# DeNA/Chainer_Realtime_Multi-Person_Pose_Estimation

Hardware: AMD Instinct MI355X
Metric: frames/sec at 368x368 batch (1/2/4/8 GPU) + keypoint-match vs reference (higher is better)
Workload: dtype f32; 1 GPU; batch32_368x368_synthetic_uint8_per_gpu; per_gpu_batch=32, global_batch=32, map=320x320, weights=seeded He + calibrated head, records_gathered=32, status_bits=0

## Files before the change

### chainer_realtime_multi-person_pose_estimation_amd/csrc/conv1_wino.hip

```cpp
#include <type_traits>
#include "pmx_common.h"
#include "wino_util.h"

#ifndef PMX_C1W_ABLATE
#define PMX_C1W_ABLATE 0
#endif
namespace {
constexpr int TT = 8;
constexpr int HW1 = 2 * TT + 2;
constexpr int NPX = HW1 * HW1;
constexpr int PW = HW1 + 2, PPX = PW * PW;
constexpr int LDA = 68;
constexpr int LDU = 36;
constexpr int U_HALF = 4 * 64 * LDU;
constexpr int RAW_ELEMS = NPX * LDA, U_ELEMS = 2 * U_HALF;
constexpr int LDS_BYTES = (RAW_ELEMS + U_ELEMS + 64) * 4;
static_assert(LDS_BYTES <= 160 * 1024, "conv1 Winograd kernel: LDS");
static_assert(PPX * 3 <= U_ELEMS, "the input patch lives in U before the first transform");
}

__global__ __launch_bounds__(256, 1) void conv1_wino_kernel(const ConvArgs a)
{
    extern __shared__ float4 smem4[];
    float* const s_raw = reinterpret_cast<float*>(smem4);
    float* const s_u = s_raw + RAW_ELEMS;
    float* const s_bias = s_u + U_ELEMS;
    float* const s_patch = s_u;
    const int tid = threadIdx.x, lane = tid & 63, wave = tid >> 6, li = lane & 31, kh = lane >> 5;
    const int th = wave >> 1, chh = wave & 1;
    int tile;
    {
        const int nwg = gridDim.x, bid = blockIdx.x;
        const int q = nwg >> 3, r = nwg & 7, xcd = bid & 7, loc = bid >> 3;
        tile = (xcd < r ? xcd * (q + 1) : r * (q + 1) + (xcd - r) * q) + loc;
    }
    int H = a.H, W = a.W, s_tiles_x = a.tiles_x, tiles_per_img = a.tiles_x * a.tiles_y;
    size_t s_pix_in = 0, s_pix_out = 0;
    if (a.nseg > 0) {
        int sg = 0;
        for (int k = 1; k < a.nseg; ++k) sg = tile >= a.segs[k].tile0 ? k : sg;
        const ConvSeg S = a.segs[sg];
        H = S.H; W = S.W; s_tiles_x = S.tiles_x; tiles_per_img = S.tiles_img;
        s_pix_in = (size_t)(unsigned)S.pix0; s_pix_out = (size_t)(unsigned)S.pixo;
        tile -= S.tile0;
    }
    const int bimg = tile / tiles_per_img;
    const int trem = tile - bimg * tiles_per_img;
    const int y0 = (trem / s_tiles_x) * (2 * TT), x0 = (trem % s_tiles_x) * (2 * TT);
    constexpr int OUTSIDE = (int)0x80000000;

    if (a.g[1].in) {
        const uint8_t* src8 = reinterpret_cast<const uint8_t*>(a.g[1].in) + (s_pix_in + (size_t)bimg * H * W) * 3;
        const __amdgpu_buffer_rsrc_t irsrc = __builtin_amdgcn_make_buffer_rsrc(const_cast<uint8_t*>(src8), 0, (unsigned)(H * W * 3), 0x00020000);
        const float divisor = __builtin_bit_cast(float, (unsigned)a.kbounds);
        unsigned char pb[2][3];
        bool pin[2];
#pragma unroll
        for (int r = 0; r < 2; ++r) {
            const int f = tid + r * 256;
            const int py = f / PW, px = f - py * PW;
            const int gy = y0 - 2 + py, gx = x0 - 2 + px;
            pin[r] = f < PPX && (unsigned)gy < (unsigned)H && (unsigned)gx < (unsigned)W;
            const int o = pin[r] ? (gy * W + gx) * 3 : OUTSIDE;
#pragma unroll
            for (int ch = 0; ch < 3; ++ch) pb[r][ch] = __builtin_amdgcn_raw_buffer_load_b8(irsrc, o, ch, 0);
        }
#pragma unroll
        for (int r = 0; r < 2; ++r) {
            const int f = tid + r * 256;
            if (f < PPX) {
#pragma unroll
                for (int ch = 0; ch < 3; ++ch)
                    s_patch[f * 3 + ch] = pin[r] ? __fsub_rn(__fdiv_rn((float)pb[r][ch], divisor), 0.5f) : 0.f;
            }
        }
    } else {
        const __amdgpu_buffer_rsrc_t irsrc = __builtin_amdgcn_make_buffer_rsrc(const_cast<float*>(a.g[0].in + (s_pix_in + (size_t)bimg * H * W) * a.lda), 0,
                                                                               (unsigned)(H * W * a.lda) * 4u, 0x00020000);
        float4 pv[2];
#pragma unroll
        for (int r = 0; r < 2; ++r) {
            const int f = tid + r * 256;
            const int py = f / PW, px = f - py * PW;
            const int gy = y0 - 2 + py, gx = x0 - 2 + px;
            const bool in = f < PPX && (unsigned)gy < (unsigned)H && (unsigned)gx < (unsigned)W;
            pv[r] = __builtin_bit_cast(float4, __builtin_amdgcn_raw_buffer_load_b128(irsrc, in ? (gy * W + gx) * a.lda * 4 : OUTSIDE, 0, 0));
        }
#pragma unroll
        for (int r = 0; r < 2; ++r) {
            const int f = tid + r * 256;
            if (f < PPX) { s_patch[f * 3 + 0] = pv[r].x; s_patch[f * 3 + 1] = pv[r].y; s_patch[f * 3 + 2] = pv[r].z; }
        }
    }
    float wv[14];
    int koff[14];
    {
        const float* wp = a.g[1].w + chh * (14 * 64) + lane;
#pragma unroll
        for (int s = 0; s < 14; ++s) {
            const int k = 2 * s + kh, kk = k < 27 ? k : 26;
            wv[s] = (PMX_C1W_ABLATE & 32) ? 1.f : wp[s * 64];
            const int tap = kk / 3;
            koff[s] = ((tap / 3) * PW + tap % 3) * 3 + kk % 3;
        }
    }
    f32x4 b1[4];
#pragma unroll
    for (int q = 0; q < 4; ++q) b1[q] = *reinterpret_cast<const f32x4*>(a.g[1].bias + chh * 32 + 8 * q + 4 * kh);
    if (tid < 64) s_bias[tid] = a.g[0].bias[tid];
    const __amdgpu_buffer_rsrc_t wrsrc = __builtin_amdgcn_make_buffer_rsrc(const_cast<float*>(a.g[0].w), 0, 0x7fffffff, 0x00020000);
    const unsigned b_off = (unsigned)((chh * 1024 + li * 8 + kh * 4) * 4);
    constexpr unsigned panel_b = 64u * 32u * 4u, freq_b = panel_b * 2u;
    auto wload = [&](int g) -> f32x4 {
        const int P = g >> 4, s = g & 15;
        const unsigned so = (unsigned)(4 * (P & 3) + (s >> 2)) * freq_b + (unsigned)(P >> 2) * panel_b;
        return __builtin_bit_cast(f32x4, __builtin_amdgcn_raw_buffer_load_b128(wrsrc, b_off + (unsigned)(s & 3) * 1024u, so, 0));
    };
    f32x4 bw[16];
#pragma unroll
    for (int g = 0; g < 8; ++g) bw[g] = wload(g);
    __syncthreads();

    const float b1s = a.g[1].bias[chh * 32 + li];
    int c1_m[5], c1_pb[5];
    float c1_hi[5];
#pragma unroll
    for (int i = 0; i < 5; ++i) {
        const int m = ((wave >> 1) + 2 * i) * 32 + li;
        const int hy = m / HW1, hx = m - hy * HW1;
        c1_m[i] = m;
        c1_pb[i] = (hy * PW + hx) * 3;
        const int gy = y0 - 1 + hy, gx = x0 - 1 + hx;
        c1_hi[i] = ((unsigned)gy < (unsigned)H && (unsigned)gx < (unsigned)W) ? __builtin_inff() : 0.f;
    }
    if (!(PMX_C1W_ABLATE & 1)) {
        const f32x16 z16 = {0.f, 0.f, 0.f, 0.f, 0.f, 0.f, 0.f, 0.f, 0.f, 0.f, 0.f, 0.f, 0.f, 0.f, 0.f, 0.f};
        float pa[2][14];
        f32x16 acc1[2];
        f32x4 ev;
#pragma unroll
        for (int sg = 0; sg < 14; ++sg) pa[0][sg] = s_patch[c1_pb[0] + koff[sg]];
        auto c1_finish = [&](const f32x16& acc, int i, int sg) {
            const int q = sg / 3, part = sg - 3 * q;
            if (q >= 4) return;
            if (part == 0) ev = pk_add4(f32x4{acc[4 * q], acc[4 * q + 1], acc[4 * q + 2], acc[4 * q + 3]}, b1[q]);
            else if (part == 1) {
#pragma unroll
                for (int e = 0; e < 4; ++e) ev[e] = __builtin_amdgcn_fmed3f(ev[e], 0.f, c1_hi[i]);
            } else *reinterpret_cast<f32x4*>(&s_raw[c1_m[i] * LDA + chh * 32 + 8 * q + 4 * kh]) = ev;
        };
#pragma unroll
        for (int i = 0; i < 5; ++i) {
#pragma unroll
            for (int sg = 0; sg < 14; ++sg) {
                acc1[i & 1] = __builtin_amdgcn_mfma_f32_32x32x2f32(wv[sg], pa[i & 1][sg], sg == 0 ? z16 : acc1[i & 1], 0, 0, 0);
                if (i + 1 < 5) pa[(i + 1) & 1][sg] = s_patch[c1_pb[i + 1] + koff[sg]];
                if (i > 0) c1_finish(acc1[(i - 1) & 1], i - 1, sg);
                __builtin_amdgcn_sched_barrier(0);
            }
        }
        {
            const int p4 = 2 * (wave >> 1) + kh, m = 320 + p4;
            const int hy = m / HW1, hx = m - hy * HW1, pb = (hy * PW + hx) * 3;
            float accv = 0.f;
#pragma unroll
            for (int sg = 0; sg < 14; ++sg) {
                const float other = __shfl_xor(wv[sg], 32);
                const float we = kh ? other : wv[sg], wo = kh ? wv[sg] : other;
                const int k0 = 2 * sg, k1 = 2 * sg + 1;
                accv = __builtin_fmaf(s_patch[pb + ((k0 / 9) * PW + (k0 / 3) % 3) * 3 + k0 % 3], we, accv);
                if (k1 < 27) accv = __builtin_fmaf(s_patch[pb + ((k1 / 9) * PW + (k1 / 3) % 3) * 3 + k1 % 3], wo, accv);
            }
            const int gy = y0 - 1 + hy, gx = x0 - 1 + hx;
            const float hi = ((unsigned)gy < (unsigned)H && (unsigned)gx < (unsigned)W) ? __builtin_inff() : 0.f;
            s_raw[m * LDA + chh * 32 + li] = __builtin_amdgcn_fmed3f(accv + b1s, 0.f, hi);
        }
#pragma unroll
        for (int sg = 0; sg < 12; ++sg) c1_finish(acc1[0], 4, sg);
    }
    __syncthreads();

    const int tg = tid >> 3, tc = tid & 7;
    const int tt = (tg & ~7) + ((tg & 7) >> 1) + 4 * (tg & 1);
    int t_raw[2];
#pragma unroll
    for (int it = 0; it < 2; ++it) {
        const int t = tt + 32 * it;
        t_raw[it] = ((2 * (t >> 3)) * HW1 + 2 * (t & 7)) * LDA + tc * 4;
    }
    const int t_u = tt * LDU + tc * 4;
    auto row_a = [](int i) { return i == 0 ? 0 : i == 1 ? 1 : i == 2 ? 2 : 1; };
    auto row_b = [](int i) { return i == 0 ? 2 : i == 1 ? 2 : i == 2 ? 1 : 3; };
    f32x4 dA[2][4], dB[2][4], wq[2][4], vq[2][4];
    auto tr_read = [&](int it, int k, int ch, int i) {
        const int row = k < 4 ? row_a(i) : row_b(i), jx = k & 3;
        const f32x4 v = *reinterpret_cast<const f32x4*>(&s_raw[t_raw[it] + (row * HW1 + jx) * LDA + ch * 32]);
        if (k < 4) dA[it][jx] = v; else dB[it][jx] = v;
    };
    auto tr_w = [&](int it, int jx, int i) { wq[it][jx] = i == 1 ? pk_add4(dA[it][jx], dB[it][jx]) : pk_sub4(dA[it][jx], dB[it][jx]); };
    auto tr_v = [&](int it, int jv) {
        vq[it][jv] = jv == 0 ? pk_sub4(wq[it][0], wq[it][2]) : jv == 1 ? pk_add4(wq[it][1], wq[it][2]) : jv == 2 ? pk_sub4(wq[it][2], wq[it][1]) : pk_sub4(wq[it][1], wq[it][3]);
    };
    auto tr_store = [&](int it, int jv, int half) {
        *reinterpret_cast<f32x4*>(&s_u[half * U_HALF + (jv * 64 + 32 * it) * LDU + t_u]) = vq[it][jv];
    };
    auto side = [&](int t, int ch, int i, int half) {
        if (t < 8) tr_read(0, t, ch, i);
        else if (t < 16) {
            tr_read(1, t - 8, ch, i);
            if (t < 12) tr_w(0, t - 8, i); else tr_v(0, t - 12);
        } else if (t < 20) { tr_store(0, t - 16, half); tr_w(1, t - 16, i); }
        else if (t < 24) tr_v(1, t - 20);
        else if (t < 28) tr_store(1, t - 24, half);
    };
#pragma unroll
    for (int t = 0; t < 28; ++t) side(t, 0, 0, 0);
    __syncthreads();

    f32x16 acc[16];
    f32x4 av[4];
    const int a_off = (32 * th + li) * LDU + kh * 4;
    av[0] = *reinterpret_cast<const f32x4*>(&s_u[a_off]);
    av[1] = *reinterpret_cast<const f32x4*>(&s_u[a_off + 8]);
    const f32x16 zero16 = {0.f, 0.f, 0.f, 0.f, 0.f, 0.f, 0.f, 0.f, 0.f, 0.f, 0.f, 0.f, 0.f, 0.f, 0.f, 0.f};
    auto phase = [&](auto P_c) {
        constexpr int P = decltype(P_c)::value;
        constexpr int ch = P >> 2, i = P & 3, half = P & 1;
        constexpr int Pn = P + 1, chn = Pn >> 2, in = Pn & 3, halfn = Pn & 1;
#pragma unroll
        for (int s = 0; s < 16; ++s) {
            const int f = 4 * i + (s >> 2), g = P * 16 + s;
#pragma unroll
            for (int e = 0; e < 4; ++e) {
                acc[f] = wino_mfma(av[s & 3][e], bw[g & 15][e], (ch == 0 && (s & 3) == 0 && e == 0) ? zero16 : acc[f]);
                if (e == 0) {
                    if (g + 8 < 128 && !(PMX_C1W_ABLATE & 4)) bw[(g + 8) & 15] = wload(g + 8);
                    if (s == 14 && P < 7) __syncthreads();
                    __builtin_amdgcn_sched_barrier(0);
                } else if (e == 1) {
                    const int sn = s + 2;
                    if (sn < 16) av[sn & 3] = *reinterpret_cast<const f32x4*>(&s_u[half * U_HALF + ((sn >> 2) * 64) * LDU + a_off + (sn & 3) * 8]);
                    else if (P < 7) av[sn & 3] = *reinterpret_cast<const f32x4*>(&s_u[halfn * U_HALF + a_off + (sn & 3) * 8]);
                    __builtin_amdgcn_sched_barrier(0);
                } else {
                    if (P < 7 && !(PMX_C1W_ABLATE & 2)) side(2 * s + (e - 2), chn, in, halfn);
                    __builtin_amdgcn_sched_barrier(0);
                }
            }
        }
    };
    if (!(PMX_C1W_ABLATE & 8)) {
    phase(std::integral_constant<int, 0>{}); phase(std::integral_constant<int, 1>{}); phase(std::integral_constant<int, 2>{});
    phase(std::integral_constant<int, 3>{}); phase(std::integral_constant<int, 4>{}); phase(std::integral_constant<int, 5>{});
    phase(std::integral_constant<int, 6>{}); phase(std::integral_constant<int, 7>{});
    } else {
#pragma unroll
        for (int f = 0; f < 16; ++f) acc[f] = zero16;
    }
    __builtin_amdgcn_sched_barrier(0);
#pragma unroll
    for (int f = 0; f < 16; ++f) asm volatile("" : "+a"(acc[f]));
    __builtin_amdgcn_sched_barrier(0);

    f32x4 bq[4];
#pragma unroll
    for (int q = 0; q < 4; ++q) bq[q] = *reinterpret_cast<const f32x4*>(&s_bias[chh * 32 + 8 * q + 4 * kh]);
    float pooled[16];
#pragma unroll
    for (int rp = 0; rp < 8; ++rp) {
        f32x2 t0[4], t1[4];
#pragma unroll
        for (int j = 0; j < 4; ++j) {
            const f32x2 m0 = {acc[0 + j][2 * rp], acc[0 + j][2 * rp + 1]}, m1 = {acc[4 + j][2 * rp], acc[4 + j][2 * rp + 1]};
            const f32x2 m2 = {acc[8 + j][2 * rp], acc[8 + j][2 * rp + 1]}, m3 = {acc[12 + j][2 * rp], acc[12 + j][2 * rp + 1]};
            t0[j] = pk_add2(pk_add2(m0, m1), m2);
            t1[j] = pk_sub2(pk_sub2(m1, m2), m3);
        }
        const f32x2 o0 = pk_add2(pk_add2(t0[0], t0[1]), t0[2]), o1 = pk_sub2(pk_sub2(t0[1], t0[2]), t0[3]);
        const f32x2 o2 = pk_add2(pk_add2(t1[0], t1[1]), t1[2]), o3 = pk_sub2(pk_sub2(t1[1], t1[2]), t1[3]);
#pragma unroll
        for (int h2 = 0; h2 < 2; ++h2) pooled[2 * rp + h2] = fmaxf(fmaxf(o0[h2], o1[h2]), fmaxf(o2[h2], o3[h2]));
    }
    const int Hp = H >> 1, Wp = W >> 1, ldc_b = a.ldc * 4;
    const __amdgpu_buffer_rsrc_t orsrc = __builtin_amdgcn_make_buffer_rsrc(a.g[0].out + (s_pix_out + (size_t)bimg * Hp * Wp) * a.ldc, 0, (unsigned)(Hp * Wp * ldc_b), 0x00020000);
    const int tb = 32 * th + li;
    const int py = (y0 >> 1) + (tb >> 3), px = (x0 >> 1) + (tb & 7);
    const int o = (py < Hp && px < Wp) ? (int)__umul24(__umul24(py, Wp) + px, ldc_b) + (chh * 32 + 4 * kh) * 4 : OUTSIDE;
    const float lo = a.relu ? 0.f : -__builtin_inff();
    typedef unsigned u32x4 __attribute__((ext_vector_type(4)));
#pragma unroll
    for (int q = 0; q < 4; ++q) {
        f32x4 v;
#pragma unroll
        for (int e = 0; e < 4; ++e) v[e] = fmaxf(pooled[4 * q + e] + bq[q][e], lo);
        if (PMX_C1W_ABLATE & 16) asm volatile("" :: "v"(v));
        else __builtin_amdgcn_raw_buffer_store_b128(__builtin_bit_cast(u32x4, v), orsrc, o + q * 32, 0, 0);
    }
}

int conv1_wino_launch(const ConvArgs& a0, hipStream_t stream)
{
    ConvArgs a = a0;
    PMX_CHECK(a.cout_pad == 64 && a.g[0].cout == 64 && a.nch == 4 && a.lda >= 4 && a.pool && a.ldc % 4 == 0, PMX_ERR_INVALID,
              "conv1 winograd: needs conv1_2 = 64 -> 64 with the pool and a >= 4-channel padded input");
    PMX_CHECK(a.H % 2 == 0 && a.W % 2 == 0, PMX_ERR_INVALID, "conv: pooled layer needs even H, W");
    PMX_CHECK((long long)a.H * a.W * a.lda * 4 < (1ll << 31) && (long long)a.H * a.W * a.ldc < (1ll << 31), PMX_ERR_INVALID, "conv: image too large for 32-bit offsets");
    a.tiles_x = (a.W + 2 * TT - 1) / (2 * TT);
    a.tiles_y = (a.H + 2 * TT - 1) / (2 * TT);
    a.ksplit = 1;
    if (!a.g[1].in) a.kbounds = 0;
    static bool attr_set[PMX_MAX_DEVICES] = {};
    if (int rc = conv_allow_big_lds(reinterpret_cast<const void*>(conv1_wino_kernel), attr_set)) return rc;
    PMX_CHECK(a.nseg == 0 || (a.segs && a.seg_tiles > 0), PMX_ERR_INVALID, "conv1 winograd: segments without a table");
    hipLaunchKernelGGL(conv1_wino_kernel, dim3(a.nseg ? (unsigned)a.seg_tiles : (unsigned)(a.tiles_x * a.tiles_y * a.B)), dim3(256), LDS_BYTES, stream, a);
    PMX_HIP(hipGetLastError());
    return PMX_OK;
}
```

Baseline: 960.1 frames/s.

## Swizzle conv1 raw tile LDS layout, issue weight loads before patch staging

Drops the padded LDA=68 row stride for an unpadded stride of 64 with an XOR swizzle of the 16-byte chunk index. The conv1 MFMA stores and the Winograd transform reads both use it, keeping LDS access conflict-free while shrinking the buffer. The filter-transform weight prefetch now issues before the input patch load so their latencies overlap. The scalar tail for pixels 320-323 is replaced by an extra MFMA tile on waves with th==0. This adds redundant MFMA work on half the waves, creates wave divergence, and makes the index math more complex.

New measurement: 955.6 frames/s. No clear change (-0.5%).

```diff
diff --git a/chainer_realtime_multi-person_pose_estimation_amd/csrc/conv1_wino.hip b/chainer_realtime_multi-person_pose_estimation_amd/csrc/conv1_wino.hip
--- a/chainer_realtime_multi-person_pose_estimation_amd/csrc/conv1_wino.hip
+++ b/chainer_realtime_multi-person_pose_estimation_amd/csrc/conv1_wino.hip
@@ -10,13 +10,15 @@
 constexpr int HW1 = 2 * TT + 2;
 constexpr int NPX = HW1 * HW1;
 constexpr int PW = HW1 + 2, PPX = PW * PW;
-constexpr int LDA = 68;
+constexpr int LDA = 64;
+constexpr int NT1 = (NPX + 31) / 32;
 constexpr int LDU = 36;
 constexpr int U_HALF = 4 * 64 * LDU;
 constexpr int RAW_ELEMS = NPX * LDA, U_ELEMS = 2 * U_HALF;
 constexpr int LDS_BYTES = (RAW_ELEMS + U_ELEMS + 64) * 4;
 static_assert(LDS_BYTES <= 160 * 1024, "conv1 Winograd kernel: LDS");
 static_assert(PPX * 3 <= U_ELEMS, "the input patch lives in U before the first transform");
+__device__ __forceinline__ int c1w_swz(int m) { return ((m & 1) << 2) | (m & 2) | (((m >> 2) & 1) * 9); }
 }
 
 __global__ __launch_bounds__(256, 1) void conv1_wino_kernel(const ConvArgs a)
@@ -26,7 +28,7 @@
     float* const s_u = s_raw + RAW_ELEMS;
     float* const s_bias = s_u + U_ELEMS;
     float* const s_patch = s_u;
-    const int tid = threadIdx.x, lane = tid & 63, wave = tid >> 6, li = lane & 31, kh = lane >> 5;
+    const int tid = threadIdx.x, lane = tid & 63, wave = __builtin_amdgcn_readfirstlane(tid >> 6), li = lane & 31, kh = lane >> 5;
     const int th = wave >> 1, chh = wave & 1;
     int tile;
     {
@@ -49,49 +51,6 @@
     const int y0 = (trem / s_tiles_x) * (2 * TT), x0 = (trem % s_tiles_x) * (2 * TT);
     constexpr int OUTSIDE = (int)0x80000000;
 
-    if (a.g[1].in) {
-        const uint8_t* src8 = reinterpret_cast<const uint8_t*>(a.g[1].in) + (s_pix_in + (size_t)bimg * H * W) * 3;
-        const __amdgpu_buffer_rsrc_t irsrc = __builtin_amdgcn_make_buffer_rsrc(const_cast<uint8_t*>(src8), 0, (unsigned)(H * W * 3), 0x00020000);
-        const float divisor = __builtin_bit_cast(float, (unsigned)a.kbounds);
-        unsigned char pb[2][3];
-        bool pin[2];
-#pragma unroll
-        for (int r = 0; r < 2; ++r) {
-            const int f = tid + r * 256;
-            const int py = f / PW, px = f - py * PW;
-            const int gy = y0 - 2 + py, gx = x0 - 2 + px;
-            pin[r] = f < PPX && (unsigned)gy < (unsigned)H && (unsigned)gx < (unsigned)W;
-            const int o = pin[r] ? (gy * W + gx) * 3 : OUTSIDE;
-#pragma unroll
-            for (int ch = 0; ch < 3; ++ch) pb[r][ch] = __builtin_amdgcn_raw_buffer_load_b8(irsrc, o, ch, 0);
-        }
-#pragma unroll
-        for (int r = 0; r < 2; ++r) {
-            const int f = tid + r * 256;
-            if (f < PPX) {
-#pragma unroll
-                for (int ch = 0; ch < 3; ++ch)
-                    s_patch[f * 3 + ch] = pin[r] ? __fsub_rn(__fdiv_rn((float)pb[r][ch], divisor), 0.5f) : 0.f;
-            }
-        }
-    } else {
-        const __amdgpu_buffer_rsrc_t irsrc = __builtin_amdgcn_make_buffer_rsrc(const_cast<float*>(a.g[0].in + (s_pix_in + (size_t)bimg * H * W) * a.lda), 0,
-                                                                               (unsigned)(H * W * a.lda) * 4u, 0x00020000);
-        float4 pv[2];
-#pragma unroll
-        for (int r = 0; r < 2; ++r) {
-            const int f = tid + r * 256;
-            const int py = f / PW, px = f - py * PW;
-            const int gy = y0 - 2 + py, gx = x0 - 2 + px;
-            const bool in = f < PPX && (unsigned)gy < (unsigned)H && (unsigned)gx < (unsigned)W;
-            pv[r] = __builtin_bit_cast(float4, __builtin_amdgcn_raw_buffer_load_b128(irsrc, in ? (gy * W + gx) * a.lda * 4 : OUTSIDE, 0, 0));
-        }
-#pragma unroll
-        for (int r = 0; r < 2; ++r) {
-            const int f = tid + r * 256;
-            if (f < PPX) { s_patch[f * 3 + 0] = pv[r].x; s_patch[f * 3 + 1] = pv[r].y; s_patch[f * 3 + 2] = pv[r].z; }
-        }
-    }
     float wv[14];
     int koff[14];
     {
@@ -107,7 +66,7 @@
     f32x4 b1[4];
 #pragma unroll
     for (int q = 0; q < 4; ++q) b1[q] = *reinterpret_cast<const f32x4*>(a.g[1].bias + chh * 32 + 8 * q + 4 * kh);
-    if (tid < 64) s_bias[tid] = a.g[0].bias[tid];
+    const float b2v = a.g[0].bias[tid & 63];
     const __amdgpu_buffer_rsrc_t wrsrc = __builtin_amdgcn_make_buffer_rsrc(const_cast<float*>(a.g[0].w), 0, 0x7fffffff, 0x00020000);
     const unsigned b_off = (unsigned)((chh * 1024 + li * 8 + kh * 4) * 4);
     constexpr unsigned panel_b = 64u * 32u * 4u, freq_b = panel_b * 2u;
@@ -119,16 +78,61 @@
     f32x4 bw[16];
 #pragma unroll
     for (int g = 0; g < 8; ++g) bw[g] = wload(g);
+    __builtin_amdgcn_sched_barrier(0);
+    if (a.g[1].in) {
+        const uint8_t* src8 = reinterpret_cast<const uint8_t*>(a.g[1].in) + (s_pix_in + (size_t)bimg * H * W) * 3;
+        const __amdgpu_buffer_rsrc_t irsrc = __builtin_amdgcn_make_buffer_rsrc(const_cast<uint8_t*>(src8), 0, (unsigned)(H * W * 3), 0x00020000);
+        const float divisor = __builtin_bit_cast(float, (unsigned)a.kbounds);
+        unsigned char pb[2][3];
+        bool pin[2];
+#pragma unroll
+        for (int r = 0; r < 2; ++r) {
+            const int f = tid + r * 256;
+            const int py = f / PW, px = f - py * PW;
+            const int gy = y0 - 2 + py, gx = x0 - 2 + px;
+            pin[r] = f < PPX && (unsigned)gy < (unsigned)H && (unsigned)gx < (unsigned)W;
+            const int o = pin[r] ? (gy * W + gx) * 3 : OUTSIDE;
+#pragma unroll
+            for (int ch = 0; ch < 3; ++ch) pb[r][ch] = __builtin_amdgcn_raw_buffer_load_b8(irsrc, o, ch, 0);
+        }
+#pragma unroll
+        for (int r = 0; r < 2; ++r) {
+            const int f = tid + r * 256;
+            if (f < PPX) {
+#pragma unroll
+                for (int ch = 0; ch < 3; ++ch)
+                    s_patch[f * 3 + ch] = pin[r] ? __fsub_rn(__fdiv_rn((float)pb[r][ch], divisor), 0.5f) : 0.f;
+            }
+        }
+    } else {
+        const __amdgpu_buffer_rsrc_t irsrc = __builtin_amdgcn_make_buffer_rsrc(const_cast<float*>(a.g[0].in + (s_pix_in + (size_t)bimg * H * W) * a.lda), 0,
+                                                                               (unsigned)(H * W * a.lda) * 4u, 0x00020000);
+        float4 pv[2];
+#pragma unroll
+        for (int r = 0; r < 2; ++r) {
+            const int f = tid + r * 256;
+            const int py = f / PW, px = f - py * PW;
+            const int gy = y0 - 2 + py, gx = x0 - 2 + px;
+            const bool in = f < PPX && (unsigned)gy < (unsigned)H && (unsigned)gx < (unsigned)W;
+            pv[r] = __builtin_bit_cast(float4, __builtin_amdgcn_raw_buffer_load_b128(irsrc, in ? (gy * W + gx) * a.lda * 4 : OUTSIDE, 0, 0));
+        }
+#pragma unroll
+        for (int r = 0; r < 2; ++r) {
+            const int f = tid + r * 256;
+            if (f < PPX) { s_patch[f * 3 + 0] = pv[r].x; s_patch[f * 3 + 1] = pv[r].y; s_patch[f * 3 + 2] = pv[r].z; }
+        }
+    }
+    if (tid < 64) s_bias[tid] = b2v;
     __syncthreads();
 
-    const float b1s = a.g[1].bias[chh * 32 + li];
-    int c1_m[5], c1_pb[5];
-    float c1_hi[5];
-#pragma unroll
-    for (int i = 0; i < 5; ++i) {
-        const int m = ((wave >> 1) + 2 * i) * 32 + li;
-        const int hy = m / HW1, hx = m - hy * HW1;
-        c1_m[i] = m;
+    constexpr int NI = (NT1 + 1) / 2;
+    int c1_w[NI], c1_pb[NI];
+    float c1_hi[NI];
+#pragma unroll
+    for (int i = 0; i < NI; ++i) {
+        const int m = (th + 2 * i) * 32 + li, mc = m < NPX ? m : NPX - 1;
+        const int hy = mc / HW1, hx = mc - hy * HW1;
+        c1_w[i] = m < NPX ? m * LDA + (((chh * 8 + kh) ^ c1w_swz(m)) << 2) : -1;
         c1_pb[i] = (hy * PW + hx) * 3;
         const int gy = y0 - 1 + hy, gx = x0 - 1 + hx;
         c1_hi[i] = ((unsigned)gy < (unsigned)H && (unsigned)gx < (unsigned)W) ? __builtin_inff() : 0.f;
@@ -147,54 +151,48 @@
             else if (part == 1) {
 #pragma unroll
                 for (int e = 0; e < 4; ++e) ev[e] = __builtin_amdgcn_fmed3f(ev[e], 0.f, c1_hi[i]);
-            } else *reinterpret_cast<f32x4*>(&s_raw[c1_m[i] * LDA + chh * 32 + 8 * q + 4 * kh]) = ev;
+            } else if (i < NI - 1 || c1_w[i] >= 0) *reinterpret_cast<f32x4*>(&s_raw[c1_w[i] ^ (8 * q)]) = ev;
         };
-#pragma unroll
-        for (int i = 0; i < 5; ++i) {
+        auto c1_tile = [&](int i) {
 #pragma unroll
             for (int sg = 0; sg < 14; ++sg) {
                 acc1[i & 1] = __builtin_amdgcn_mfma_f32_32x32x2f32(wv[sg], pa[i & 1][sg], sg == 0 ? z16 : acc1[i & 1], 0, 0, 0);
-                if (i + 1 < 5) pa[(i + 1) & 1][sg] = s_patch[c1_pb[i + 1] + koff[sg]];
+                if (i + 1 < NI) pa[(i + 1) & 1][sg] = s_patch[c1_pb[i + 1] + koff[sg]];
                 if (i > 0) c1_finish(acc1[(i - 1) & 1], i - 1, sg);
                 __builtin_amdgcn_sched_barrier(0);
             }
-        }
-        {
-            const int p4 = 2 * (wave >> 1) + kh, m = 320 + p4;
-            const int hy = m / HW1, hx = m - hy * HW1, pb = (hy * PW + hx) * 3;
-            float accv = 0.f;
-#pragma unroll
-            for (int sg = 0; sg < 14; ++sg) {
-                const float other = __shfl_xor(wv[sg], 32);
-                const float we = kh ? other : wv[sg], wo = kh ? wv[sg] : other;
-                const int k0 = 2 * sg, k1 = 2 * sg + 1;
-                accv = __builtin_fmaf(s_patch[pb + ((k0 / 9) * PW + (k0 / 3) % 3) * 3 + k0 % 3], we, accv);
-                if (k1 < 27) accv = __builtin_fmaf(s_patch[pb + ((k1 / 9) * PW + (k1 / 3) % 3) * 3 + k1 % 3], wo, accv);
-            }
-            const int gy = y0 - 1 + hy, gx = x0 - 1 + hx;
-            const float hi = ((unsigned)gy < (unsigned)H && (unsigned)gx < (unsigned)W) ? __builtin_inff() : 0.f;
-            s_raw[m * LDA + chh * 32 + li] = __builtin_amdgcn_fmed3f(accv + b1s, 0.f, hi);
-        }
-#pragma unroll
-        for (int sg = 0; sg < 12; ++sg) c1_finish(acc1[0], 4, sg);
+        };
+#pragma unroll
+        for (int i = 0; i < NI - 1; ++i) c1_tile(i);
+        if (th == 0) {
+            c1_tile(NI - 1);
+#pragma unroll
+            for (int sg = 0; sg < 12; ++sg) c1_finish(acc1[(NI - 1) & 1], NI - 1, sg);
+        } else {
+#pragma unroll
+            for (int sg = 0; sg < 12; ++sg) c1_finish(acc1[(NI - 2) & 1], NI - 2, sg);
+        }
     }
     __syncthreads();
 
     const int tg = tid >> 3, tc = tid & 7;
-    const int tt = (tg & ~7) + ((tg & 7) >> 1) + 4 * (tg & 1);
-    int t_raw[2];
+    const int tt = (tg & ~7) + ((tg & 7) ^ ((tg >> 1) & 1));
+    int t_raw[2], t_sw[8];
 #pragma unroll
     for (int it = 0; it < 2; ++it) {
         const int t = tt + 32 * it;
-        t_raw[it] = ((2 * (t >> 3)) * HW1 + 2 * (t & 7)) * LDA + tc * 4;
-    }
+        t_raw[it] = ((2 * (t >> 3)) * HW1 + 2 * (t & 7)) * LDA;
+    }
+#pragma unroll
+    for (int j = 0; j < 8; ++j) t_sw[j] = (tc ^ c1w_swz((2 * (tt >> 3)) * HW1 + 2 * (tt & 7) + j)) << 2;
     const int t_u = tt * LDU + tc * 4;
     auto row_a = [](int i) { return i == 0 ? 0 : i == 1 ? 1 : i == 2 ? 2 : 1; };
     auto row_b = [](int i) { return i == 0 ? 2 : i == 1 ? 2 : i == 2 ? 1 : 3; };
     f32x4 dA[2][4], dB[2][4], wq[2][4], vq[2][4];
     auto tr_read = [&](int it, int k, int ch, int i) {
         const int row = k < 4 ? row_a(i) : row_b(i), jx = k & 3;
-        const f32x4 v = *reinterpret_cast<const f32x4*>(&s_raw[t_raw[it] + (row * HW1 + jx) * LDA + ch * 32]);
+        const int d = row * HW1 + jx;
+        const f32x4 v = *reinterpret_cast<const f32x4*>(&s_raw[t_raw[it] + d * LDA + (t_sw[d & 7] ^ (ch * 32))]);
         if (k < 4) dA[it][jx] = v; else dB[it][jx] = v;
     };
     auto tr_w = [&](int it, int jx, int i) { wq[it][jx] = i == 1 ? pk_add4(dA[it][jx], dB[it][jx]) : pk_sub4(dA[it][jx], dB[it][jx]); };
```
